# waiwera/waiwera

Hardware: AMD Instinct MI355X
Metric: Newton steps/sec, 10M-cell eos_we (BCSR SpMV GB/s in roofline) (higher is better)
Workload: dtype f64

## Files before the change

### include/waiwera_hip_bench.h

```cpp
#ifndef WAIWERA_HIP_BENCH_H
#define WAIWERA_HIP_BENCH_H
#include "waiwera_hip.h"
#ifdef __cplusplus
extern "C" {
#endif

int wai_comm_stats(wai_ctx *ctx, long long *allreduces, long long *exchanges);
int wai_gather_stats(wai_ctx *ctx, long long *gathers);
int wai_launch_stats(wai_ctx *ctx, long long *kernels, long long *copies);
int wai_tracer_stats(wai_ctx *ctx, long long *assembly_sweeps);

int wai_bench_mute_comm(wai_ctx *ctx, int on);
int wai_test_drop_partials(wai_ctx *ctx, int n);
int wai_test_drop_stream_wait(wai_ctx *ctx, int which);
int wai_test_network_pass(wai_ctx *ctx, const double *raw2n, double *sources6, double *groups6, double *reinjectors8,
                          double *net2n, double *enth_n);
int wai_test_network_stats(wai_ctx *ctx, long long *passes, long long *host_waits);
int wai_test_coupling_build_stats(wai_ctx *ctx, long long *launches, long long *columns, long long *chunks);
int wai_test_network_lds(wai_ctx *ctx, int *limit, int *needed);
int wai_test_device_memory(long long *allocations, long long *bytes);
int wai_test_pc_operator(wai_ctx *ctx, int spmv, const double *x, const double *x2, double alpha, int dot_mode,
                         const double *aux, int split, int fin_phase, const double *scal_in, double *z, double *scal_out);
int wai_pc_axpy_capable(wai_ctx *ctx);
int wai_test_partial_count(wai_ctx *ctx);
int wai_test_desc_templates(wai_ctx *ctx, int *bricks, int *rows);
int wai_test_pack_groups(wai_ctx *ctx, int list, int *shared, int *table, int cap);
int wai_test_tile_schedule(wai_ctx *ctx, int extended, int *facts);
enum { WAI_KV_DOT = 0, WAI_KV_DOTS, WAI_KV_WAXPY, WAI_KV_BCGS_P, WAI_KV_BCGS_S, WAI_KV_BCGS_XR, WAI_KV_BCGS_XRP,
       WAI_KV_BCGS_XRP_DERIVE, WAI_KV_SCALARS, WAI_KV_MDOT, WAI_KV_MAXPY_NORM, WAI_KV_SCALE_TO, WAI_KV_UPDATE_X };
int wai_test_krylov_vec(wai_ctx *ctx, int op, int variant, int n, int k, long long ld, long long len, double alpha,
                        double *vecs, double *basis, const double *coef, double *scal, double *post);
int wai_halo_size(wai_ctx *ctx, int dof, long long *bytes_sent, int *n_neighbours);

int wai_timer_start(wai_ctx *ctx);
int wai_timer_stop(wai_ctx *ctx, float *ms);
int wai_bench_kernel(wai_ctx *ctx, int which, int reps, float *ms_per_launch);
int wai_bcgs_composed(wai_ctx *ctx);
int wai_profile_enable(wai_ctx *ctx, int on);
int wai_profile_get(wai_ctx *ctx, int kclass, double *ms, long long *launches);
// ... 7 lines not shown
```

### waiwera_amd/csrc/capi.hip

```cpp
#include "host.hpp"

using namespace wai;

namespace wai {

int fetch_flags(wai_ctx* c, int out[4]) {
  if (c->comm && c->comm->nranks > 1) {
    HIPCHK(c, hipMemcpyAsync(c->h_flags, c->d_flags, 4 * sizeof(int), hipMemcpyDeviceToHost, c->stream));
    HIPCHK(c, hipStreamSynchronize(c->stream));
    double v[4] = {(double)c->h_flags[0], -(double)c->h_flags[1], (double)c->h_flags[2], (double)c->h_flags[3]};
    HIPCHK(c, hipMemcpyAsync(c->d_red + 2048, v, sizeof(v), hipMemcpyHostToDevice, c->stream));
    if (comm_allreduce(c->comm, c->d_red + 2048, 4, 1, c->stream, c->err)) return -1;
    HIPCHK(c, hipMemcpyAsync(c->h_red + 8, c->d_red + 2048, sizeof(v), hipMemcpyDeviceToHost, c->stream));
    HIPCHK(c, hipStreamSynchronize(c->stream));
    out[0] = (int)c->h_red[8]; out[1] = c->h_flags[1]; out[2] = (int)c->h_red[10]; out[3] = (int)c->h_red[11];
  } else {
    HIPCHK(c, hipMemcpyAsync(c->h_flags, c->d_flags, 4 * sizeof(int), hipMemcpyDeviceToHost, c->stream));
    HIPCHK(c, hipStreamSynchronize(c->stream));
    for (int i = 0; i < 4; i++) out[i] = c->h_flags[i];
  }
  HIPCHK(c, hipMemcpyAsync(c->d_flags, FLAGS_RESET, sizeof(FLAGS_RESET), hipMemcpyHostToDevice, c->stream));
  return 0;
}

// ... 10 lines not shown
  }
  int fl[4];
  if (fetch_flags(c, fl)) return -1;
  return fl[0] ? 1 : 0;
}

int do_residual(wai_ctx* c, double dt, double* y, const double* lhs_old, double* f) {
  int e = do_pre_eval(c, y);
  if (e) return e;
  if (c->net.on && network_update(c)) return -1;
  Prof p(c, KC_RESIDUAL);
  launch_residual(c, dt, lhs_old, f, nullptr, nullptr);
  return 0;
}

int do_jacobian(wai_ctx* c, double dt, const double* y, const double* lhs_old) {
  {
    Prof p(c, KC_EOS);
    launch_eos(c, y, 0, c->mesh.n_prim, true);
  }
  int fl[4];
  if (fetch_flags(c, fl)) return -1;
  if (fl[0]) return 1;
  Prof p(c, KC_JACOBIAN);
  if (launch_jacobian(c, dt, lhs_old)) return -1;
  pc_invalidate(c, c->flow);
  return network_couplings(c, dt, const_cast<double*>(y), lhs_old);
}

int do_norm2(wai_ctx* c, const double* v, double* out) {
  vec_dot(c, v, v, c->flow.n, S_W2);
  if (allreduce_scal(c, S_W2, 1)) return -1;
  if (read_scal(c, S_W2, 1)) return -1;
  *out = std::sqrt(c->ks.h_scal[S_W2]);
  return 0;
}

int do_max_scaled(wai_ctx* c, const double* v, const double* scale, double tol, double* val, int* idx) {
  if (launch_max_scaled(c, v, scale, tol, val, idx)) return -1;
  if (c->comm && c->comm->nranks > 1) {
// ... 385 lines not shown
```

### waiwera_amd/csrc/context.hip

```cpp
#include "host.hpp"
#include "cell_order.hpp"
#include <cstdio>

using namespace wai;

namespace wai {

int alloc_krylov_vecs(wai_ctx* c, KrylovVecs& k, size_t nl) {
  for (auto p : {&k.R, &k.RP, &k.P, &k.V, &k.S, &k.T, &k.tmp, &k.X_own})
    if (!*p && p->alloc_zeroed(c, nl + 16)) return -1;
  k.X = k.X_own;
  return 0;
}
int ensure_basis(wai_ctx* c, LinSys& sys, int m) {
  KrylovVecs& k = *sys.kv;
  if (k.basis && k.basis_m >= m) return 0;
  k.basis_m = m;
  return k.basis.alloc_zeroed(c, (size_t)(m + 4) * sys.nl);
}
int ensure_bcgsl_vecs(wai_ctx* c, KrylovVecs& k, size_t nl) {
  if (k.bl) return 0;
  return k.bl.alloc_zeroed(c, BCGSL_VECS * (nl + 16));
}
Bcsr matrix_on(const Pattern& p, int bs, double* val) {
// ... 2 lines not shown
  A.bs = bs; A.val = val;
  return A;
}
static KspOpts ksp_of(const wai_solver_opts& o) {
  KspOpts k;
  k.type = o.ksp_type; k.restart = o.gmres_restart; k.max_its = o.ksp_max_its; k.rtol = o.ksp_rtol; k.atol = o.ksp_atol;
  return k;
}

Handles::~Handles() {
  for (hipEvent_t e : {ev0, ev1, ev_scal, ev_pack, ev_halo}) if (e) (void)hipEventDestroy(e);
  if (comm_stream) (void)hipStreamDestroy(comm_stream);
  for (hipEvent_t e : {pev0, pev1}) if (e) (void)hipEventDestroy(e);
  if (stream) (void)hipStreamDestroy(stream);
  comm_destroy(comm);
}

}

static int create_handles(wai_ctx* c, int device) {
  c->device = device;
  HIPCHK(c, hipSetDevice(device));
  {
    int ncu = 0;
    if (hipDeviceGetAttribute(&ncu, hipDeviceAttributeMultiprocessorCount, device) == hipSuccess && ncu > 0) c->n_cu = ncu;
    int lds = 0;
    if (hipDeviceGetAttribute(&lds, hipDeviceAttributeMaxSharedMemoryPerBlock, device) == hipSuccess && lds > 0) c->lds_per_block = (size_t)lds;
  }
  HIPCHK(c, hipStreamCreateWithFlags(&c->stream, hipStreamNonBlocking));
  HIPCHK(c, hipEventCreate(&c->ev0)); HIPCHK(c, hipEventCreate(&c->ev1));
// ... 96 lines not shown
    std::vector<int> cs(N, -1);
    if (c->mesh.cell_src.upload(c, cs)) return -1;
  }
  std::vector<int> sub;
  if (md->sub_ptr && md->n_sub > 0) sub.assign(md->sub_ptr, md->sub_ptr + md->n_sub + 1);
  else sub = {0, N};
  return build_schedule(c, c->ilu, J.h_rowptr, J.h_colidx, sub, N, J.W, np, true);
}

static int create_vectors(wai_ctx* c) {
  const DeviceMesh& m = c->mesh;
  const int NL = m.n_local, np = c->np;
  LinSys& flow = c->flow;
  const size_t nl = (size_t)np * m.n_prim, n = (size_t)np * m.n_owned;
  const size_t fsz = (size_t)c->df * NL;
  if (c->flu.alloc_zeroed(c, fsz) || c->flu_last_iter.alloc(c, fsz) || c->flu_last_step.alloc(c, fsz) ||
      c->flu_pert.alloc(c, (size_t)np * c->df * m.n_prim) || c->hstep.alloc(c, nl))
    return -1;
  {
    std::vector<double> ones(NL, 1.0);
    HIPCHK(c, hipMemcpy(c->flu + (size_t)F_REGION * NL, ones.data(), NL * sizeof(double), hipMemcpyHostToDevice));
    HIPCHK(c, hipMemcpy(c->flu + (size_t)F_OLD_REGION * NL, ones.data(), NL * sizeof(double), hipMemcpyHostToDevice));
  }
  for (auto p : {&c->w_y, &c->w_yold, &c->w_delta, &c->w_f, &c->w_lhs, &c->w_a, &c->w_b, &c->w_c, &c->w_lhs2, &c->w_hist,
                 &c->w_hist_prev})
    if (p->alloc_zeroed(c, nl + 16)) return -1;
  flow.n = (int)n; flow.nl = (int)nl;
  if (alloc_krylov_vecs(c, c->kv, nl)) return -1;
  if (c->opts.gmres_restart > MAX_RESTART) { c->err = "gmres restart above 40 is not supported"; return -2; }
  c->kv.basis_m = basis_vectors(c->opts.gmres_restart);
  if ((flow.ksp.type == WAI_KSP_GMRES || flow.ksp.type == WAI_KSP_LGMRES) && ensure_basis(c, flow, c->kv.basis_m)) return -1;
  return 0;
// ... 321 lines not shown
```

### waiwera_amd/csrc/context.hpp

```cpp
#pragma once
#include <hip/hip_runtime.h>
#include <string>
#include <type_traits>
#include <vector>
#include "../../include/waiwera_hip.h"
#include "colour_order.hpp"
#include "coupling_batch.hpp"
#include "devbuf.hpp"
#include "ilu_schedule.hpp"
#include "mesh_pattern.hpp"
#include "network_pass.hpp"
#include "network_wave.hpp"
#include "physics.hip.h"
#include "tile_schedule.hpp"

namespace wai {

__host__ __device__ __forceinline__ size_t ell_ld(size_t n) {
  size_t ld = (n + 511) & ~(size_t)511;
  if ((ld & 262143) == 0) ld += 512;
  return ld;
}
__host__ __device__ __forceinline__ size_t ell_rows(int bs, size_t n) {
  if (bs >= 3) return ell_ld(n);
// ... 400 lines not shown
  wai::DevBuf<double> w_hist;
  wai::DevBuf<double> w_hist_prev;
  double dt_last_prev = 0.0;
  bool can_reject = false;
  bool prof_on = false;
  bool last_iter_partial = false;
  double prof_ms[wai::KC_COUNT] = {0};
  long long prof_n[wai::KC_COUNT] = {0};
  std::string err;
  bool bc_set = false;
  int dbg = 0;
};

namespace wai {
int launch_eos(wai_ctx* c, const double* y, int first, int count, bool perturbed);
int launch_residual(wai_ctx* c, double dt, const double* lhs_old, double* f, double* lhs_out,
                    double* rhs_out, const int* only = nullptr, int n_only = 0);
int launch_jacobian(wai_ctx* c, double dt, const double* lhs_old);
int launch_transitions(wai_ctx* c, const double* y_old, double* search, double* y);
int launch_tracer_assemble(wai_ctx* c, const TracerForm& tf, const double* alx_last,
                           const double* alx_last2, double* b);
int launch_tracer_assemble_all(wai_ctx* c, int method, double dt, double ratio, const double* alx_last,
                               const double* alx_last2, double* b);
int launch_tracer_lhs(wai_ctx* c, double* Al);
int launch_separator(wai_ctx* c, double pressure, double* out);
int launch_face_fluxes(wai_ctx* c, const int* face_cells, double* out);
int launch_source_rates(wai_ctx* c, double* out, bool raw = false);
int launch_network_pass(wai_ctx* c, const double* raw, double* net, double* enth, double* state_out, bool wave);
int net_wave_allow_lds(wai_ctx* c, const void* kernel, int bit, size_t* bytes);
int launch_cp_perturb(wai_ctx* c, double* p, double* yh);
int launch_cp_restore(wai_ctx* c, double* p, const double* yh);
int launch_cp_diff(wai_ctx* c, int ml, int m, int bs, int j, int k, const double* g, const double* yh, double* val, int* flag);
int launch_coupling_batch(wai_ctx* c, const CouplingBatch& b, int col0, int ncol, double dt, const double* y, const double* lhs_old,
// ... 70 lines not shown
```

### waiwera_amd/csrc/kernels_factor.hip

```cpp
#include "linalg_device.hip.h"
#include "pc_lu.hip.h"

namespace wai {

template <int BS>
__global__ void k_ilu_factor(int n, int nsub, const int* __restrict__ sub_ptr,
                             const int* __restrict__ sub_nlev, const int* __restrict__ row_info,
                             const int* __restrict__ col, double* fval, double* __restrict__ dinv,
                             int* flags) {
  constexpr int BB = BS * BS;
  const int s = xcd_remap(blockIdx.x, nsub);
  if (s >= nsub) return;
  const int lo = sub_ptr[s], R = sub_ptr[s + 1] - lo;
  const int nlf = sub_nlev[s] & 0xffff;
  const int i = lo + threadIdx.x;
  const bool active = (int)threadIdx.x < R;
  int lfirst = 0, dslot = 0, ulast = 0, lf = -1, lb = 0;
  if (active) unpack_info(row_info[i], lfirst, dslot, ulast, lf, lb);
  for (int lev = 0; lev < nlf; lev++) {
    if (active && lf == lev) {
      for (int q = lfirst; q < dslot; q++) {
        const int k = col[(size_t)q * n + i];
        int kl, kd, ku, kf, kb;
        unpack_info(row_info[k], kl, kd, ku, kf, kb);
// ... 109 lines not shown
      double piv[BB], inv[BB];
#pragma unroll
      for (int z = 0; z < BB; z++) piv[z] = fval[vix<BS>(n, dslot, z, i)];
      if (!block_inverse<BS>(piv, inv)) atomicMax(&flags[0], 1);
#pragma unroll
      for (int z = 0; z < BB; z++) {
        fval[vix<BS>(n, dslot, z, i)] = inv[z];
        dinv[dix<BS>(n, z, i)] = inv[z];
      }
    }
    __threadfence_block();
    __syncthreads();
  }
}

template <int BS, bool PRE>
__global__ void k_dilu_pivots(int n, int nsub, const int* __restrict__ sub_ptr,
                              const int* __restrict__ sub_nlev, const int* __restrict__ row_info,
                              const int* __restrict__ col, const double* __restrict__ aval,
                              double* __restrict__ dinv, int* flags) {
  constexpr int BB = BS * BS;
  extern __shared__ double pinv[];
  const int s = xcd_remap(blockIdx.x, nsub);
  if (s >= nsub) return;
  const int lo = sub_ptr[s], R = sub_ptr[s + 1] - lo;
  const int nlf = sub_nlev[s] & 0xffff;
  const int tid = threadIdx.x, i = lo + tid;
  const bool active = tid < R;
  int lfirst = 0, dslot = 0, ulast = 0, lf = -1, lb = 0;
  double P[BB];
#pragma unroll
  for (int e = 0; e < BB; e++) P[e] = 0.0;
  if (active) {
    unpack_info(row_info[i], lfirst, dslot, ulast, lf, lb);
    load_block<BS>(aval, n, dslot, i, P);
  }
  constexpr int NP = PRE ? 3 : 1;
  double paik[NP][BB], paki[NP][BB];
  int pk_off[NP];
  if constexpr (PRE) {
#pragma unroll
    for (int p = 0; p < NP; p++) {
      pk_off[p] = -1;
#pragma unroll
      for (int e = 0; e < BB; e++) { paik[p][e] = 0.0; paki[p][e] = 0.0; }
      const int q = lfirst + p;
      if (active && q < dslot) {
        const int k = col[(size_t)q * n + i];
        int kl, kd, ku, kf, kb;
        unpack_info(row_info[k], kl, kd, ku, kf, kb);
        load_block<BS>(aval, n, q, i, paik[p]);
// ... 41 lines not shown
          for (int e = 0; e < BB; e++) aki[e] = 0.0;
          for (int r2 = kd + 1; r2 < ku; r2++)
            if (col[(size_t)r2 * n + k] == i) { load_block<BS>(aval, n, r2, k, aki); break; }
          update(aik, pinv + (size_t)(k - lo) * BB, aki);
        }
      }
      double inv[BB];
      if (!block_inverse<BS>(P, inv)) atomicMax(&flags[0], 1);
#pragma unroll
      for (int e = 0; e < BB; e++) {
        pinv[(size_t)tid * BB + e] = inv[e];
        dinv[dix<BS>(n, e, i)] = inv[e];
      }
    }
    __syncthreads();
  }
}

template <int BS, int NPL, bool RAIK>
__global__ __launch_bounds__(256) void k_dilu_pivots_lds(int n, int nsub, int cap, const int* __restrict__ sub_ptr,
                                  const int* __restrict__ sub_nlev, const int* __restrict__ row_info,
                                  const int* __restrict__ row_tslot, const int* __restrict__ col,
                                  const double* __restrict__ aval, double* __restrict__ dinv, int* flags) {
  constexpr int BB = BS * BS;
  extern __shared__ double sm[];
  const int s = xcd_remap(blockIdx.x, nsub);
  if (s >= nsub) return;
  const int lo = sub_ptr[s], R = sub_ptr[s + 1] - lo;
  const int nlf = sub_nlev[s] & 0xffff;
  const int tid = threadIdx.x, i = lo + tid;
// ... 79 lines not shown
    __syncthreads();
  }
}

template <int BS>
__global__ __launch_bounds__(TPB) void k_scale_rows(int n, int W, const double* __restrict__ aval,
                                                    const double* __restrict__ dinv, double* __restrict__ sval) {
  constexpr int BB = BS * BS;
  const int i = blockIdx.x * TPB + threadIdx.x;
  if (i >= n) return;
  double d[BB];
  load_pivot<BS>(dinv, n, i, d);
  for (int q = 0; q < W; q++) {
    double a[BB];
    load_block<BS>(aval, n, q, i, a);
#pragma unroll
    for (int r = 0; r < BS; r++)
#pragma unroll
      for (int c = 0; c < BS; c++) {
        double t = 0.0;
#pragma unroll
        for (int e = 0; e < BS; e++) t += d[r * BS + e] * a[e * BS + c];
        sval[vix<BS>(n, q, r * BS + c, i)] = t;
      }
  }
}

template <int BS>
__global__ __launch_bounds__(TPB) void k_lvl_factor(int n, int cnt, const int* __restrict__ ord,
                                                    const int* __restrict__ row_info, const int* __restrict__ col,
                                                    double* fval, double* __restrict__ dinv, int* flags) {
  constexpr int BB = BS * BS;
  const int t = blockIdx.x * TPB + threadIdx.x;
  if (t >= cnt) return;
  const int i = ord[t];
  int lfirst, dslot, ulast;
  unpack_info_wide(row_info[i], lfirst, dslot, ulast);
  for (int q = lfirst; q < dslot; q++) {
    const int k = col[(size_t)q * n + i];
// ... 305 lines not shown
                       s.fval, s.dinv, c->d_flags);
    return;
  }
  if (s.big) {
    hipMemcpyAsync(s.fval, J.val, sizeof(double) * ell_size(J.bs, J.n, J.W), hipMemcpyDeviceToDevice, c->stream);
    for (int lev = 0; lev < s.nlev_f; lev++) {
      const int a = s.lev_f_ptr[lev], cnt = s.lev_f_ptr[lev + 1] - a, g = (cnt + TPB - 1) / TPB;
      if (cnt <= 0) continue;
      hipLaunchKernelGGL(k_lvl_factor<BS>, g, TPB, 0, c->stream, J.n, cnt, s.ord_f + a, s.row_info, J.col, s.fval, s.dinv, c->d_flags);
    }
    return;
  }
  const int grid = ((s.nsub + 7) / 8) * 8, T = pc_threads(s);
  if (s.diag_only && s.scaled) {
    const size_t lds = (size_t)T * J.bs * J.bs * sizeof(double);
    auto pivots = [&](auto pre) {
      hipLaunchKernelGGL((k_dilu_pivots<BS, decltype(pre)::value>), grid, T, lds, c->stream, J.n, s.nsub, s.sub_ptr, s.sub_nlev,
                         s.row_info, J.col, J.val, s.dinv, c->d_flags);
    };
    if constexpr (BS <= 2) with_flag(s.fast3, pivots);
    else if constexpr (BS == 3) {
      auto staged = [&](auto npl, auto raik, size_t lds_s) {
        hipLaunchKernelGGL((k_dilu_pivots_lds<3, decltype(npl)::value, decltype(raik)::value>), grid, T, lds_s, c->stream, J.n, s.nsub,
                           s.max_rows, s.sub_ptr, s.sub_nlev, s.row_info, s.row_tslot, J.col, J.val, s.dinv, c->d_flags);
      };
      const int npl = s.max_nl <= 3 ? 3 : 4;
      const size_t lds2 = (size_t)(1 + 2 * npl) * 9 * s.max_rows * sizeof(double);
      const std::integral_constant<int, 3> three;
      if (npl == 3 && T <= 64)
        staged(three, std::true_type{}, (size_t)(1 + npl) * 9 * s.max_rows * sizeof(double));
      else if (s.max_nl <= 4 && lds2 <= 64 * 1024 && T <= 256) {
        if (npl == 3) staged(three, std::false_type{}, lds2);
        else staged(std::integral_constant<int, 4>{}, std::false_type{}, lds2);
      } else
        pivots(std::false_type{});
    } else
      pivots(std::false_type{});
    hipLaunchKernelGGL(k_scale_rows<BS>, (J.n + TPB - 1) / TPB, TPB, 0, c->stream, J.n, J.W, J.val, s.dinv, s.fval);
    return;
  }
  hipMemcpyAsync(s.fval, J.val, sizeof(double) * ell_size(J.bs, J.n, J.W), hipMemcpyDeviceToDevice, c->stream);
  if (s.wide)
    hipLaunchKernelGGL(k_ilu_factor_wide<BS>, grid, T, 0, c->stream, J.n, s.nsub, s.sub_ptr, s.sub_nlev, s.row_infow, J.col, s.fval, s.dinv, c->d_flags);
  else
    hipLaunchKernelGGL(k_ilu_factor<BS>, grid, T, 0, c->stream, J.n, s.nsub, s.sub_ptr, s.sub_nlev, s.row_info, J.col, s.fval, s.dinv, c->d_flags);
}
int launch_ilu_factor_on(wai_ctx* c, const Bcsr& J, IluSchedule& s) {
  if (J.dg) return launch_dg_factor(c, J, s);
  return with_bs(J.bs, [&](auto bs) { ilu_factor_bs<decltype(bs)::value>(c, J, s); });
}

template <int BS, bool FWD>
static void lvl_sweep(wai_ctx* c, const Bcsr& J, const IluSchedule& s, const int* ord, const std::vector<int>& ptr, int nlev, double* z) {
// ... 51 lines not shown
```

### waiwera_amd/csrc/kernels_jacobian.hip

```cpp
#include "assembly_device.hip.h"

namespace wai {

template <int KIND>
__global__ __launch_bounds__(TPB) void k_jacobian(MeshView m, const double* __restrict__ flu,
                                                  size_t stride, const double* __restrict__ flu_pert,
                                                  const double* __restrict__ hstep, int n_prim,
                                                  ResForm rf, double* __restrict__ val) {
  using E = EosT<KIND>;
  constexpr int np = E::np, bb = E::np * E::np;
  const int c = xcd_cell(m.n_owned);
  if (c < 0) return;
  CellState<KIND> own0;
  RockState rown;
  load_state<KIND>(flu, stride, c, own0);
  load_rock(m.rock, m.n_local, c, rown);
  const double vol = m.vol[c];
  double lold[np], lold2[np];
#pragma unroll
  for (int k = 0; k < np; k++) {
    lold[k] = rf.method == WAI_METHOD_DIRECTSS ? 0.0 : rf.last[(size_t)c * np + k];
    lold2[k] = rf.method == WAI_METHOD_BDF2 ? rf.last2[(size_t)c * np + k] : 0.0;
  }

// ... 381 lines not shown
  for (int k = 0; k < np; k++) { R0[k] += src0[k]; f0[k] = res_form(rf, L0[k], R0[k], lold[k], lold2[k]); }
  const int dq = m.diag_blk[c];
#pragma unroll
  for (int k = 0; k < np; k++) {
    CellState<KIND> ownk;
    unpark_state<KIND>(park + (size_t)k * nld * st + threadIdx.x, st, ownk);
    source_terms<KIND>(m, c, ownk, vol, Rk[k]);
#pragma unroll
    for (int r = 0; r < np; r++) {
      const double f1 = res_form(rf, lpark[(size_t)(k * np + r) * st], Rk[k][r], lold[r], lold2[r]);
      __builtin_nontemporal_store((f1 - f0[r]) / hk[k], val + ell_ix(np, nrow, dq, r, k, (size_t)c));
    }
  }
}

int launch_jacobian(wai_ctx* c, double dt, const double* lhs_old) {
  const MeshView m = view(c);
  const size_t stride = c->mesh.n_local;
  const ResForm rf = res_form_of(c, dt, lhs_old);
  const char* ep = getenv("WAI_JAC_PARK");
  const bool park = !(ep && ep[0] == '0');
  const char* es = getenv("WAI_JAC_SYM");
  const bool sym = park && c->mesh.adj_tblk && (es ? es[0] == '1' : true);
  const char* kernel = nullptr;
  if (with_eos(c->kind, [&](auto k) {
        constexpr int K = decltype(k)::value;
        constexpr int T = ParkT<K>::threads;
        constexpr int sym_lds = EosT<K>::np * (ParkT<K>::npark + EosT<K>::np) * 8 * T;
        const int g = (((int)((m.n_owned + T - 1) / T) + 7) / 8) * 8;
        if (sym && (size_t)sym_lds <= c->lds_per_block) {
          kernel = "k_jacobian_sym";
          hipLaunchKernelGGL(k_jacobian_sym<K>, g, T, sym_lds, c->stream, m, c->flu, stride, c->flu_pert, c->hstep,
                             c->mesh.n_prim, rf, c->flow.A.val);
          return;
        }
        if (m.max_deg > MAXDEG) {
          c->err = "the row-wise Jacobian (WAI_JAC_SYM=0) supports cells with at most 8 faces; this mesh has a cell with " +
                   std::to_string(m.max_deg) + " (the default column-wise Jacobian takes up to 16)";
          return;
        }
        if (park && ParkT<K>::use) {
// ... 14 lines not shown
```

### waiwera_amd/csrc/measure.hip

```cpp
#include "host.hpp"

using namespace wai;

namespace {
typedef double stream_d2 __attribute__((ext_vector_type(2)));
__global__ __launch_bounds__(256) void k_stream_copy(const stream_d2* __restrict__ src, stream_d2* __restrict__ dst, size_t n2) {
  const size_t stride = (size_t)gridDim.x * 256;
  size_t i = (size_t)blockIdx.x * 256 + threadIdx.x;
  for (; i + stride < n2; i += 2 * stride) {
    const stream_d2 a = __builtin_nontemporal_load(src + i), b = __builtin_nontemporal_load(src + i + stride);
    __builtin_nontemporal_store(a, dst + i);
    __builtin_nontemporal_store(b, dst + i + stride);
  }
  if (i < n2) __builtin_nontemporal_store(__builtin_nontemporal_load(src + i), dst + i);
}
__global__ __launch_bounds__(256) void k_stream_read(const stream_d2* __restrict__ src, size_t n2, double* sink) {
  const size_t stride = (size_t)gridDim.x * 256;
  size_t i = (size_t)blockIdx.x * 256 + threadIdx.x;
  double t = 0.0;
  for (; i + stride < n2; i += 2 * stride) {
    const stream_d2 a = __builtin_nontemporal_load(src + i), b = __builtin_nontemporal_load(src + i + stride);
    t += (a.x + a.y) + (b.x + b.y);
  }
  if (i < n2) { const stream_d2 a = __builtin_nontemporal_load(src + i); t += a.x + a.y; }
// ... 13 lines not shown
  KrylovVecs& k = *sys.kv;
  if ((which == 20 || which == 21) && !k.basis) { c->err = "wai_bench_kernel 20 / 21: no Krylov basis (ksp_type gmres)"; return -2; }
  if (which > 0 && c->ilu.owner != &sys) { const int e = do_pc_setup(c, sys); if (e) return e < 0 ? -1 : e; }
  if (which > 0 && pc_colour(c, sys)) { c->err = "wai_bench_kernel: the natural order's kernels, not the multicolour ordering (tools/pc_colour_timing.py times it)"; return -2; }
  const bool fill = pc_fill_fused(c, sys);
  if (which == 23 && (!pc_fused(c, sys) || !(fill ? sys.as.sched.ord_f : c->ilu.ord_f))) {
    c->err = "wai_bench_kernel 23: no level sets (a block-Jacobi schedule of a wide mesh, or fused ILU(k))";
    return -2;
  }
  if (pc_asm_fused(c, sys) && (which == 9 || which == 10 || which == 16 || which == 23)) {
    c->err = "wai_bench_kernel 9 / 10 / 16 / 23: the brick schedule's kernels and the level sets of a factor on the system's own rows, not fused PCASM";
    return -2;
  }
  if (fill && (which == 9 || which == 10 || which == 16)) { c->err = "wai_bench_kernel 9 / 10 / 16: the brick schedule's kernels, not fused ILU(k)"; return -2; }
  const size_t copy_n = (size_t)c->np * c->df * c->mesh.n_prim / 2;
  auto run = [&]() {
    switch (which) {
      case 0: launch_spmv(c, sys.A, k.P, k.tmp); break;
      case 1: case 3: pc_solve(c, sys, k.P, k.V, PC_DOT_NONE, nullptr, nullptr); break;
      case 23:
        launch_spmv(c, sys.A, k.P, k.V);
        if (fill) launch_big_solve(c, sys.as.E, sys.as.sched, k.V);
        else launch_big_solve(c, sys.A, c->ilu, k.V);
        break;
      case 9: if (c->ilu.n_int > 0) launch_pc(c, sys.A, true, k.P, k.V, PC_DOT_ZA, k.RP, c->ilu.sub_int, c->ilu.n_int); break;
      case 10: if (c->ilu.n_bnd > 0) launch_pc(c, sys.A, true, k.P, k.V, PC_DOT_ZA, k.RP, c->ilu.sub_bnd, c->ilu.n_bnd); break;
      case 16:
        if (c->ilu.n_int > 0 && c->ilu.n_bnd > 0) {
          const Fin fin = make_fin_dots(c, PC_DOT_ZA, 2);
          launch_pc_split(c, sys.A, k.P, k.V, PC_DOT_ZA, k.RP, &fin, nullptr, nullptr);
// ... 181 lines not shown
    e = pc_amul(c, sys, k.R, k.T, dot_mode, a, fin_phase, v, false);
  } else {
    e = pc_solve(c, sys, k.R, k.T, dot_mode, k.R, a, fin_phase);
  }
  if (e) return e;
  if (fin_phase == -2 && dot_mode)
    vec_finalize(c, c->ks.nb_pc, pc_dot_slot0(dot_mode), pc_dot_nslots(dot_mode), -1);
  HIPCHK(c, hipMemcpyAsync(z, k.T, n * sizeof(double), hipMemcpyDefault, c->stream));
  HIPCHK(c, hipMemcpyAsync(s, c->ks.scal, sizeof(s), hipMemcpyDeviceToHost, c->stream));
  HIPCHK(c, hipStreamSynchronize(c->stream));
  for (int i = 0; i < 16; i++) scal_out[i] = s[i];
  return 0;
}
int wai_pc_axpy_capable(wai_ctx* c) { return c ? (pc_operand_composable(c) ? 1 : 0) : -2; }
int wai_test_partial_count(wai_ctx* c) { return c ? c->ks.nb_pc : -2; }
int wai_test_desc_templates(wai_ctx* c, int* bricks, int* rows) {
  if (!c) return -2;
  const bool have = c->ilu.sub_desc != nullptr;
  if (bricks) *bricks = c->ilu.nsub;
  if (rows) *rows = have ? c->ilu.template_rows : 0;
  return have ? c->ilu.n_templates : 0;
}
int wai_test_pack_groups(wai_ctx* c, int list, int* shared, int* table, int cap) {
  if (!c || list < 0 || list > 2 || cap < 0 || (cap > 0 && !table)) return -2;
  read_env(c);
  const IluSchedule& s = c->ilu;
  const bool packed = !s.big && pc_kernel_kind(c, c->flow.A, s) == 1 && s.col16 && !c->env.no_col16 && s.sub_desc &&
                      !c->env.no_desc_share && s.pack_tab[list] && !c->env.no_pack;
  if (shared) *shared = packed ? s.n_shared[list] : 0;
  if (!packed) return 0;
// ... 128 lines not shown
```

### waiwera_amd/flow_simulation.py

```python
import ctypes as C

import numpy as np

from . import lib as _lib
from .lib import LIB, WaiError


class FlowSimulation:
    def __init__(self, mesh, eos="we", opts=None, device=0, temperature=20.0,
                 relperm=("linear", [0.0, 1.0, 0.0, 1.0]), capillary=("zero", []), thermo="iapws",
                 permeability_modifier=None, thermo_extrapolate=False):
        self.mesh = mesh
        self.eos_name = eos
        self._keep = dict(
            face_cells=_lib._i32(mesh.face_cells), face_geom=_lib._f64(mesh.face_geom),
            cell_geom=_lib._f64(mesh.cell_geom), rock=_lib._f64(mesh.rock),
            sub_ptr=_lib._i32(mesh.sub_ptr) if mesh.sub_ptr is not None else None)
        k = self._keep
        md = _lib.MeshDesc()
        md.n_owned, md.n_halo, md.n_bc, md.n_faces = mesh.n_owned, mesh.n_halo, mesh.n_bc, mesh.n_faces
        md.face_cells = k["face_cells"].ctypes.data_as(_lib.pi)
        md.face_geom = k["face_geom"].ctypes.data_as(_lib.pd)
        md.cell_geom = k["cell_geom"].ctypes.data_as(_lib.pd)
        md.rock = k["rock"].ctypes.data_as(_lib.pd)
# ... 395 lines not shown
        ai = _lib._f64(aux) if aux is not None else None
        s_in = _lib._f64(np.zeros(16) if scal_in is None else scal_in)
        assert xi.size == self.num_dof and s_in.size == 16
        z, s_out = np.zeros(self.num_dof), np.zeros(16)
        self._chk(LIB.wai_test_pc_operator(self.h, 1 if spmv else 0, _lib.ptr(xi), _lib.ptr(x2i), float(alpha), int(dot_mode),
                                           _lib.ptr(ai), 1 if split else 0, int(fin_phase), s_in.ctypes.data_as(_lib.pd),
                                           _lib.ptr(z), s_out.ctypes.data_as(_lib.pd)), "test_pc_operator")
        return z, s_out

    def pc_axpy_capable(self):
        return LIB.wai_pc_axpy_capable(self.h) == 1

    def partial_count(self):
        return self._chk(LIB.wai_test_partial_count(self.h), "test_partial_count")

    def desc_templates(self):
        nb, nr = C.c_int(0), C.c_int(0)
        nt = self._chk(LIB.wai_test_desc_templates(self.h, C.byref(nb), C.byref(nr)), "test_desc_templates")
        return nt, nb.value, nr.value

    def pack_groups(self, which=0):
        shared = C.c_int(0)
        ng = self._chk(LIB.wai_test_pack_groups(self.h, which, C.byref(shared), None, 0), "test_pack_groups")
        table = np.zeros(ng * 32, dtype=np.int32)
        if ng:
            self._chk(LIB.wai_test_pack_groups(self.h, which, C.byref(shared), table.ctypes.data_as(C.POINTER(C.c_int)), table.size),
                      "test_pack_groups")
        return ng, shared.value, table.reshape(ng, 8, 4)

    KV_OPS = ("dot", "dots", "waxpy", "bcgs_p", "bcgs_s", "bcgs_xr", "bcgs_xrp", "bcgs_xrp_derive", "scalars", "mdot",
# ... 167 lines not shown
```

### waiwera_amd/lib.py

```python
import ctypes as C
import os

import numpy as np

HERE = os.path.dirname(os.path.abspath(__file__))
LIB_PATH = os.path.join(HERE, "libwaiwera_hip.so")

EOS_W, EOS_WE, EOS_WCE, EOS_WSE, EOS_WAE, EOS_WSCE, EOS_WSAE = 0, 1, 2, 3, 4, 5, 6
EOS_KIND = {"w": EOS_W, "we": EOS_WE, "wce": EOS_WCE, "wse": EOS_WSE, "wae": EOS_WAE, "wsce": EOS_WSCE,
            "wsae": EOS_WSAE}
RP = {"fully_mobile": 0, "fully mobile": 0, "linear": 1, "pickens": 2, "corey": 3, "grant": 4,
      "van_genuchten": 5, "van genuchten": 5, "table": 6}
CP = {"zero": 0, "linear": 1, "van_genuchten": 2, "van genuchten": 2, "table": 3}
INTERP = {"linear": 0, "step": 1, "pchip": 2}
KSP = {"bcgs": 0, "gmres": 1, "bcgsl": 2, "lgmres": 3}
PC = {"bjacobi": 0, "asm": 1, "none": 2, "lu": 3}
KCLASS = ["eos", "residual", "jacobian", "spmv", "pc_apply", "pc_setup", "vector", "transitions"]

d, i32 = C.c_double, C.c_int
pd, pi = C.POINTER(C.c_double), C.POINTER(C.c_int)


THERMO = {"iapws": 0, "ifc67": 1}
TRACER_SOLVE = {"per_tracer": 0, "coupled": 1}
# ... 116 lines not shown
        "wai_comm_init": (i32, [vp, i32, i32, C.c_char_p]),
        "wai_halo_exchange": (i32, [vp, vp, i32]),
        "wai_comm_size": (i32, [vp]),
        "wai_comm_stats": (i32, [vp, C.POINTER(C.c_longlong), C.POINTER(C.c_longlong)]),
        "wai_gather_stats": (i32, [vp, C.POINTER(C.c_longlong)]),
        "wai_gather_rows": (i32, [vp, i32, i32, vp, i32, vp, i32, vp]),
        "wai_gather_fluid": (i32, [vp, i32, i32, i32, pi, vp, i32, vp]),
        "wai_launch_stats": (i32, [vp, C.POINTER(C.c_longlong), C.POINTER(C.c_longlong)]),
        "wai_bench_mute_comm": (i32, [vp, i32]),
        "wai_test_drop_partials": (i32, [vp, i32]),
        "wai_test_drop_stream_wait": (i32, [vp, i32]),
        "wai_test_device_memory": (i32, [C.POINTER(C.c_longlong), C.POINTER(C.c_longlong)]),
        "wai_test_pc_operator": (i32, [vp, i32, vp, vp, d, i32, vp, i32, i32, pd, vp, pd]),
        "wai_pc_axpy_capable": (i32, [vp]),
        "wai_test_partial_count": (i32, [vp]),
        "wai_test_desc_templates": (i32, [vp, C.POINTER(i32), C.POINTER(i32)]),
        "wai_test_pack_groups": (i32, [vp, i32, C.POINTER(i32), C.POINTER(i32), i32]),
        "wai_test_tile_schedule": (i32, [vp, i32, C.POINTER(i32)]),
        "wai_test_krylov_vec": (i32, [vp, i32, i32, i32, i32, C.c_longlong, C.c_longlong, d, pd, pd, pd, pd, pd]),
        "wai_halo_size": (i32, [vp, i32, C.POINTER(C.c_longlong), C.POINTER(i32)]),
        "wai_pc_kernel_name": (C.c_char_p, [vp]),
        "wai_pre_timestep": (i32, [vp]),
        "wai_pre_retry_timestep": (i32, [vp]),
        "wai_pre_iteration": (i32, [vp]),
        "wai_pre_eval": (i32, [vp, d, vp]),
        "wai_lhs": (i32, [vp, d, vp, vp]),
        "wai_rhs": (i32, [vp, d, vp, vp]),
        "wai_post_linesearch": (i32, [vp, vp, vp, vp, pi, pi]),
        "wai_set_residual_form": (i32, [vp, i32, d, vp]),
        "wai_set_timestep_method": (i32, [vp, i32]),
# ... 202 lines not shown
```

Measured before the change: 5.394.

## Fuse row scaling into DILU pivot kernel and add lane-parallel Jacobian path

Folds the diagonal-inverse row scaling into the pivot kernel. Blocks already held in registers are reused, so the separate k_scale_rows pass and its reload of the matrix are skipped; this is on by default. Adds an opt-in Jacobian kernel that computes perturbed EOS states per lane inside the Jacobian itself, removing the separate perturbed EOS launch and the flu_pert buffer; this only runs when WAI_JAC_LANES=1. flu_pert is now allocated lazily, and test hooks are added for reading back the factor. The fused pivot kernel carries more register pressure, which could lower occupancy.

```diff
diff --git a/include/waiwera_hip_bench.h b/include/waiwera_hip_bench.h
--- a/include/waiwera_hip_bench.h
+++ b/include/waiwera_hip_bench.h
@@ -23,6 +23,8 @@
                          const double *aux, int split, int fin_phase, const double *scal_in, double *z, double *scal_out);
 int wai_pc_axpy_capable(wai_ctx *ctx);
 int wai_test_partial_count(wai_ctx *ctx);
+int wai_test_pc_factor(wai_ctx *ctx, long long cap_fval, double *fval, long long cap_dinv, double *dinv, int *scaled);
+int wai_test_pc_factor_size(wai_ctx *ctx, long long *n_fval, long long *n_dinv);
 int wai_test_desc_templates(wai_ctx *ctx, int *bricks, int *rows);
 int wai_test_pack_groups(wai_ctx *ctx, int list, int *shared, int *table, int cap);
 int wai_test_tile_schedule(wai_ctx *ctx, int extended, int *facts);
diff --git a/waiwera_amd/csrc/capi.hip b/waiwera_amd/csrc/capi.hip
--- a/waiwera_amd/csrc/capi.hip
+++ b/waiwera_amd/csrc/capi.hip
@@ -48,16 +48,29 @@
   return 0;
 }
 
+static std::string eos_range_message(int cell) {
+  return "FD Jacobian: a perturbed state of cell " + std::to_string(cell) + " is outside the range of the equation of state";
+}
+
 int do_jacobian(wai_ctx* c, double dt, const double* y, const double* lhs_old) {
+  int fl[4];
+  if (jacobian_lanes(c)) {
+    Prof p(c, KC_JACOBIAN);
+    if (launch_jacobian(c, dt, y, lhs_old)) return -1;
+    pc_invalidate(c, c->flow);
+    if (fetch_flags(c, fl)) return -1;
+    if (fl[0]) { c->err = eos_range_message(fl[1]); return 1; }
+    return network_couplings(c, dt, const_cast<double*>(y), lhs_old);
+  }
+  if (need_flu_pert(c)) return -1;
   {
     Prof p(c, KC_EOS);
     launch_eos(c, y, 0, c->mesh.n_prim, true);
   }
-  int fl[4];
   if (fetch_flags(c, fl)) return -1;
-  if (fl[0]) return 1;
+  if (fl[0]) { c->err = eos_range_message(fl[1]); return 1; }
   Prof p(c, KC_JACOBIAN);
-  if (launch_jacobian(c, dt, lhs_old)) return -1;
+  if (launch_jacobian(c, dt, y, lhs_old)) return -1;
   pc_invalidate(c, c->flow);
   return network_couplings(c, dt, const_cast<double*>(y), lhs_old);
 }
diff --git a/waiwera_amd/csrc/context.hip b/waiwera_amd/csrc/context.hip
--- a/waiwera_amd/csrc/context.hip
+++ b/waiwera_amd/csrc/context.hip
@@ -40,6 +40,11 @@
   for (hipEvent_t e : {pev0, pev1}) if (e) (void)hipEventDestroy(e);
   if (stream) (void)hipStreamDestroy(stream);
   comm_destroy(comm);
+}
+
+int need_flu_pert(wai_ctx* c) {
+  if (c->flu_pert) return 0;
+  return c->flu_pert.alloc(c, (size_t)c->np * c->df * c->mesh.n_prim);
 }
 
 }
@@ -166,8 +171,7 @@
   LinSys& flow = c->flow;
   const size_t nl = (size_t)np * m.n_prim, n = (size_t)np * m.n_owned;
   const size_t fsz = (size_t)c->df * NL;
-  if (c->flu.alloc_zeroed(c, fsz) || c->flu_last_iter.alloc(c, fsz) || c->flu_last_step.alloc(c, fsz) ||
-      c->flu_pert.alloc(c, (size_t)np * c->df * m.n_prim) || c->hstep.alloc(c, nl))
+  if (c->flu.alloc_zeroed(c, fsz) || c->flu_last_iter.alloc(c, fsz) || c->flu_last_step.alloc(c, fsz) || c->hstep.alloc(c, nl))
     return -1;
   {
     std::vector<double> ones(NL, 1.0);
diff --git a/waiwera_amd/csrc/context.hpp b/waiwera_amd/csrc/context.hpp
--- a/waiwera_amd/csrc/context.hpp
+++ b/waiwera_amd/csrc/context.hpp
@@ -438,9 +438,11 @@
 
 namespace wai {
 int launch_eos(wai_ctx* c, const double* y, int first, int count, bool perturbed);
+int need_flu_pert(wai_ctx* c);
+bool jacobian_lanes(const wai_ctx* c);
 int launch_residual(wai_ctx* c, double dt, const double* lhs_old, double* f, double* lhs_out,
                     double* rhs_out, const int* only = nullptr, int n_only = 0);
-int launch_jacobian(wai_ctx* c, double dt, const double* lhs_old);
+int launch_jacobian(wai_ctx* c, double dt, const double* y, const double* lhs_old);
 int launch_transitions(wai_ctx* c, const double* y_old, double* search, double* y);
 int launch_tracer_assemble(wai_ctx* c, const TracerForm& tf, const double* alx_last,
                            const double* alx_last2, double* b);
diff --git a/waiwera_amd/csrc/kernels_factor.hip b/waiwera_amd/csrc/kernels_factor.hip
--- a/waiwera_amd/csrc/kernels_factor.hip
+++ b/waiwera_amd/csrc/kernels_factor.hip
@@ -147,11 +147,23 @@
   }
 }
 
-template <int BS, bool PRE>
+template <int BS>
+__device__ __forceinline__ void scale_block(const double* d, const double* a, double* __restrict__ sval, int n, int q, int i) {
+#pragma unroll
+  for (int r = 0; r < BS; r++)
+#pragma unroll
+    for (int c = 0; c < BS; c++) {
+      double t = 0.0;
+#pragma unroll
+      for (int e = 0; e < BS; e++) t += d[r * BS + e] * a[e * BS + c];
+      sval[vix<BS>(n, q, r * BS + c, i)] = t;
+    }
+}
+template <int BS, bool PRE, bool SCALE>
 __global__ void k_dilu_pivots(int n, int nsub, const int* __restrict__ sub_ptr,
                               const int* __restrict__ sub_nlev, const int* __restrict__ row_info,
                               const int* __restrict__ col, const double* __restrict__ aval,
-                              double* __restrict__ dinv, int* flags) {
+                              double* __restrict__ dinv, int* flags, int W, double* __restrict__ sval) {
   constexpr int BB = BS * BS;
   extern __shared__ double pinv[];
   const int s = xcd_remap(blockIdx.x, nsub);
@@ -168,6 +180,11 @@
     unpack_info(row_info[i], lfirst, dslot, ulast, lf, lb);
     load_block<BS>(aval, n, dslot, i, P);
   }
+  double adiag[PRE && SCALE ? BB : 1];
+  if constexpr (PRE && SCALE) {
+#pragma unroll
+    for (int e = 0; e < BB; e++) adiag[e] = P[e];
+  }
   constexpr int NP = PRE ? 3 : 1;
   double paik[NP][BB], paki[NP][BB];
   int pk_off[NP];
@@ -239,6 +256,32 @@
       }
     }
     __syncthreads();
+  }
+  if constexpr (SCALE) {
+    if (!active) return;
+    double d[BB];
+#pragma unroll
+    for (int e = 0; e < BB; e++) d[e] = pinv[(size_t)tid * BB + e];
+    for (int q = 0; q < W; q++) {
+      double a[BB];
+      bool held = false;
+      if constexpr (PRE) {
+        if (q == dslot) {
+          held = true;
+#pragma unroll
+          for (int e = 0; e < BB; e++) a[e] = adiag[e];
+        }
+#pragma unroll
+        for (int p = 0; p < NP; p++)
+          if (q == lfirst + p && q < dslot) {
+            held = true;
+#pragma unroll
+            for (int e = 0; e < BB; e++) a[e] = paik[p][e];
+          }
+      }
+      if (!held) load_block<BS>(aval, n, q, i, a);
+      scale_block<BS>(d, a, sval, n, q, i);
+    }
   }
 }
 
@@ -348,15 +391,7 @@
   for (int q = 0; q < W; q++) {
     double a[BB];
     load_block<BS>(aval, n, q, i, a);
-#pragma unroll
-    for (int r = 0; r < BS; r++)
-#pragma unroll
-      for (int c = 0; c < BS; c++) {
-        double t = 0.0;
-#pragma unroll
-        for (int e = 0; e < BS; e++) t += d[r * BS + e] * a[e * BS + c];
-        sval[vix<BS>(n, q, r * BS + c, i)] = t;
-      }
+    scale_block<BS>(d, a, sval, n, q, i);
   }
 }
 
@@ -692,9 +727,15 @@
   const int grid = ((s.nsub + 7) / 8) * 8, T = pc_threads(s);
   if (s.diag_only && s.scaled) {
     const size_t lds = (size_t)T * J.bs * J.bs * sizeof(double);
+    const char* ef = getenv("WAI_PIVOT_SCALE");
+    const bool fuse = !(ef && ef[0] == '0');
+    bool scaled_rows = false;
     auto pivots = [&](auto pre) {
-      hipLaunchKernelGGL((k_dilu_pivots<BS, decltype(pre)::value>), grid, T, lds, c->stream, J.n, s.nsub, s.sub_ptr, s.sub_nlev,
-                         s.row_info, J.col, J.val, s.dinv, c->d_flags);
+      with_flag(fuse, [&](auto sc) {
+        hipLaunchKernelGGL((k_dilu_pivots<BS, decltype(pre)::value, decltype(sc)::value>), grid, T, lds, c->stream, J.n, s.nsub, s.sub_ptr,
+                           s.sub_nlev, s.row_info, J.col, J.val, s.dinv, c->d_flags, J.W, s.fval);
+      });
+      scaled_rows = fuse;
     };
     if constexpr (BS <= 2) with_flag(s.fast3, pivots);
     else if constexpr (BS == 3) {
@@ -714,7 +755,8 @@
         pivots(std::false_type{});
     } else
       pivots(std::false_type{});
-    hipLaunchKernelGGL(k_scale_rows<BS>, (J.n + TPB - 1) / TPB, TPB, 0, c->stream, J.n, J.W, J.val, s.dinv, s.fval);
+    if (!scaled_rows)
+      hipLaunchKernelGGL(k_scale_rows<BS>, (J.n + TPB - 1) / TPB, TPB, 0, c->stream, J.n, J.W, J.val, s.dinv, s.fval);
     return;
   }
   hipMemcpyAsync(s.fval, J.val, sizeof(double) * ell_size(J.bs, J.n, J.W), hipMemcpyDeviceToDevice, c->stream);
diff --git a/waiwera_amd/csrc/kernels_jacobian.hip b/waiwera_amd/csrc/kernels_jacobian.hip
--- a/waiwera_amd/csrc/kernels_jacobian.hip
+++ b/waiwera_amd/csrc/kernels_jacobian.hip
@@ -419,7 +419,122 @@
   }
 }
 
-int launch_jacobian(wai_ctx* c, double dt, const double* lhs_old) {
+template <int KIND> struct LanesT {
+#if defined(WAI_JAC_LANES_G2)
+  static constexpr int G = EosT<KIND>::np == 2 ? WAI_JAC_LANES_G2 : EosT<KIND>::np + 1;
+#else
+  static constexpr int G = EosT<KIND>::np + 1;
+#endif
+  static constexpr int per_wave = 64 / G;
+  static constexpr int threads = 256;
+  static constexpr int cells = (threads / 64) * per_wave;
+#if defined(WAI_JAC_LANES_WAVES)
+  static constexpr int waves = WAI_JAC_LANES_WAVES;
+#else
+  static constexpr int waves = 2;
+#endif
+};
+template <int KIND>
+__device__ __forceinline__ void as_loaded(CellState<KIND>& s) {
+  using E = EosT<KIND>;
+  s.region = 0.0;
+#pragma unroll
+  for (int q = 0; q < E::nc; q++) s.pp[q] = 0.0;
+  if constexpr (E::nc == 1) {
+#pragma unroll
+    for (int p = 0; p < E::nph; p++) s.x[p][0] = (((int)s.phases >> p) & 1) ? 1.0 : 0.0;
+  }
+}
+template <int KIND>
+__global__ __launch_bounds__(LanesT<KIND>::threads, LanesT<KIND>::waves) void k_jacobian_lanes(MeshView m, EosParams ep, const double* __restrict__ y,
+                                                  const double* __restrict__ flu, size_t stride, double eps, double umin,
+                                                  ResForm rf, double* __restrict__ val, int* flags) {
+  using E = EosT<KIND>;
+  using LT = LanesT<KIND>;
+  constexpr int np = E::np, G = LT::G;
+  const int nblk = (m.n_owned + LT::cells - 1) / LT::cells;
+  const int per = (nblk + 7) >> 3;
+  const int b = ((int)blockIdx.x & 7) * per + ((int)blockIdx.x >> 3);
+  if (((int)blockIdx.x >> 3) >= per || b >= nblk) return;
+  const int lane = (int)threadIdx.x & 63, grp = lane / G, role = lane - grp * G;
+  const int c = b * LT::cells + ((int)threadIdx.x >> 6) * LT::per_wave + grp;
+  if (grp >= LT::per_wave || role > np || c >= m.n_owned) return;
+  const int base = lane - role;
+  const int k = role - 1;
+  CellState<KIND> own;
+  RockState rown;
+  load_rock(m.rock, m.n_local, c, rown);
+  const double vol = m.vol[c];
+  double h = 1.0;
+  if (role == 0) load_state<KIND>(flu, stride, c, own);
+  else {
+    double yc[np];
+#pragma unroll
+    for (int q = 0; q < np; q++) yc[q] = y[(size_t)c * np + q];
+#pragma unroll
+    for (int q = 0; q < np; q++)
+      if (q == k) { h = fd_step(yc[q], eps, umin); yc[q] += h; }
+    const int region = (int)flu[F_REGION * stride + c];
+    if (eos_eval<KIND>(ep, yc, region, own)) flag_error(flags, c);
+    as_loaded<KIND>(own);
+  }
+  const size_t nrow = m.n_owned;
+  const double dR = res_dR(rf);
+  double L[np], R[np];
+  cell_balance<KIND>(own, rown, L);
+#pragma unroll
+  for (int q = 0; q < np; q++) R[q] = 0.0;
+#pragma unroll 1
+  for (int s = 0; s < m.max_deg; s++) {
+    const int fs = m.adj_face[(size_t)s * m.n_owned + c];
+    if (fs < 0) continue;
+    const int o = m.adj_other[(size_t)s * m.n_owned + c];
+    const int tb = m.adj_tblk[(size_t)s * m.n_owned + c];
+    FaceGeom g;
+    load_face(m, fs >> 1, g);
+    CellState<KIND> oth;
+    RockState roth;
+    load_state<KIND>(flu, stride, o, oth);
+    load_rock_face(m.rock, m.n_local, o, g.dir, roth);
+    const int side = fs & 1;
+    const double sign = side ? 1.0 : -1.0;
+    const double volo = tb >= 0 ? m.vol[o] : 1.0;
+    double fl[np];
+    slot_flux<KIND>(g, side, own, rown, oth, roth, fl);
+#pragma unroll
+    for (int q = 0; q < np; q++) R[q] += sign * (fl[q] * g.area) / vol;
+#pragma unroll
+    for (int r = 0; r < np; r++) {
+      const double to = -sign * (fl[r] * g.area) / volo;
+      const double to0 = __shfl(to, base);
+      if (role > 0 && tb >= 0) val[ell_ix(np, nrow, tb, r, k, (size_t)o)] = dR * (to - to0) / h;
+    }
+  }
+  double acc[np];
+#pragma unroll
+  for (int q = 0; q < np; q++) acc[q] = role == 0 ? 0.0 : R[q];
+  source_terms<KIND>(m, c, own, vol, acc);
+#pragma unroll
+  for (int q = 0; q < np; q++) R[q] = role == 0 ? R[q] + acc[q] : acc[q];
+  const int dq = m.diag_blk[c];
+#pragma unroll
+  for (int r = 0; r < np; r++) {
+    const double l1 = rf.method == WAI_METHOD_DIRECTSS ? 0.0 : rf.last[(size_t)c * np + r];
+    const double l2 = rf.method == WAI_METHOD_BDF2 ? rf.last2[(size_t)c * np + r] : 0.0;
+    const double f = res_form(rf, L[r], R[r], l1, l2);
+    const double f0 = __shfl(f, base);
+    if (role > 0) __builtin_nontemporal_store((f - f0) / h, val + ell_ix(np, nrow, dq, r, k, (size_t)c));
+  }
+}
+
+bool jacobian_lanes(const wai_ctx* c) {
+  const char* ep = getenv("WAI_JAC_PARK");
+  const char* es = getenv("WAI_JAC_SYM");
+  const char* el = getenv("WAI_JAC_LANES");
+  return !(ep && ep[0] == '0') && c->mesh.adj_tblk && c->mesh.n_halo == 0 && !(es && es[0] != '1') && (el && el[0] == '1');
+}
+
+int launch_jacobian(wai_ctx* c, double dt, const double* y, const double* lhs_old) {
   const MeshView m = view(c);
   const size_t stride = c->mesh.n_local;
   const ResForm rf = res_form_of(c, dt, lhs_old);
@@ -428,8 +543,18 @@
   const char* es = getenv("WAI_JAC_SYM");
   const bool sym = park && c->mesh.adj_tblk && (es ? es[0] == '1' : true);
   const char* kernel = nullptr;
+  const bool lanes = jacobian_lanes(c);
+  if (!lanes && !c->flu_pert) { c->err = "launch_jacobian: the perturbed fluid records (flu_pert) are not allocated"; return -1; }
   if (with_eos(c->kind, [&](auto k) {
         constexpr int K = decltype(k)::value;
+        if (lanes) {
+          using LT = LanesT<K>;
+          const int gl = (((int)((m.n_owned + LT::cells - 1) / LT::cells) + 7) / 8) * 8;
+          kernel = "k_jacobian_lanes";
+          hipLaunchKernelGGL(k_jacobian_lanes<K>, gl, LT::threads, 0, c->stream, m, c->ep, y, c->flu, stride, c->opts.fd_eps,
+                             c->opts.fd_umin, rf, c->flow.A.val, c->d_flags);
+          return;
+        }
         constexpr int T = ParkT<K>::threads;
         constexpr int sym_lds = EosT<K>::np * (ParkT<K>::npark + EosT<K>::np) * 8 * T;
         const int g = (((int)((m.n_owned + T - 1) / T) + 7) / 8) * 8;
diff --git a/waiwera_amd/csrc/measure.hip b/waiwera_amd/csrc/measure.hip
--- a/waiwera_amd/csrc/measure.hip
+++ b/waiwera_amd/csrc/measure.hip
@@ -51,6 +51,7 @@
   }
   if (fill && (which == 9 || which == 10 || which == 16)) { c->err = "wai_bench_kernel 9 / 10 / 16: the brick schedule's kernels, not fused ILU(k)"; return -2; }
   const size_t copy_n = (size_t)c->np * c->df * c->mesh.n_prim / 2;
+  if ((which == 18 || which == 19 || which == 22) && need_flu_pert(c)) return -1;
   auto run = [&]() {
     switch (which) {
       case 0: launch_spmv(c, sys.A, k.P, k.tmp); break;
@@ -262,6 +263,25 @@
 }
 int wai_pc_axpy_capable(wai_ctx* c) { return c ? (pc_operand_composable(c) ? 1 : 0) : -2; }
 int wai_test_partial_count(wai_ctx* c) { return c ? c->ks.nb_pc : -2; }
+int wai_test_pc_factor_size(wai_ctx* c, long long* n_fval, long long* n_dinv) {
+  if (!c || !n_fval || !n_dinv) return -2;
+  const Bcsr& J = c->flow.A;
+  *n_fval = (long long)ell_size(J.bs, J.n, J.W);
+  *n_dinv = (long long)J.n * J.bs * J.bs;
+  return 0;
+}
+int wai_test_pc_factor(wai_ctx* c, long long cap_fval, double* fval, long long cap_dinv, double* dinv, int* scaled) {
+  if (!c || cap_fval < 0 || cap_dinv < 0 || (cap_fval > 0 && !fval) || (cap_dinv > 0 && !dinv)) return -2;
+  const Bcsr& J = c->flow.A;
+  const IluSchedule& s = c->ilu;
+  if (!s.fval || !s.dinv) { c->err = "wai_test_pc_factor: no block ILU factor (wai_pc_setup first)"; return -1; }
+  const size_t nf = ell_size(J.bs, J.n, J.W), nd = (size_t)J.n * J.bs * J.bs;
+  if (scaled) *scaled = (s.diag_only && s.scaled) ? 1 : 0;
+  HIPCHK(c, hipStreamSynchronize(c->stream));
+  if (cap_fval > 0) HIPCHK(c, hipMemcpy(fval, s.fval, std::min((size_t)cap_fval, nf) * sizeof(double), hipMemcpyDeviceToHost));
+  if (cap_dinv > 0) HIPCHK(c, hipMemcpy(dinv, s.dinv, std::min((size_t)cap_dinv, nd) * sizeof(double), hipMemcpyDeviceToHost));
+  return 0;
+}
 int wai_test_desc_templates(wai_ctx* c, int* bricks, int* rows) {
   if (!c) return -2;
   const bool have = c->ilu.sub_desc != nullptr;
diff --git a/waiwera_amd/flow_simulation.py b/waiwera_amd/flow_simulation.py
--- a/waiwera_amd/flow_simulation.py
+++ b/waiwera_amd/flow_simulation.py
@@ -433,6 +433,16 @@
     def partial_count(self):
         return self._chk(LIB.wai_test_partial_count(self.h), "test_partial_count")
 
+    def pc_factor(self):
+        nf, nd, sc = C.c_longlong(0), C.c_longlong(0), C.c_int(0)
+        self._chk(LIB.wai_test_pc_factor_size(self.h, C.byref(nf), C.byref(nd)), "test_pc_factor_size")
+        fval, dinv = np.zeros(nf.value), np.zeros(nd.value)
+        self._chk(LIB.wai_test_pc_factor(self.h, nf.value, _lib.ptr(fval), nd.value, _lib.ptr(dinv), C.byref(sc)), "test_pc_factor")
+        return fval, dinv, bool(sc.value)
+
+    def last_error(self):
+        return LIB.wai_last_error(self.h).decode()
+
     def desc_templates(self):
         nb, nr = C.c_int(0), C.c_int(0)
         nt = self._chk(LIB.wai_test_desc_templates(self.h, C.byref(nb), C.byref(nr)), "test_desc_templates")
diff --git a/waiwera_amd/lib.py b/waiwera_amd/lib.py
--- a/waiwera_amd/lib.py
+++ b/waiwera_amd/lib.py
@@ -154,6 +154,8 @@
         "wai_test_pc_operator": (i32, [vp, i32, vp, vp, d, i32, vp, i32, i32, pd, vp, pd]),
         "wai_pc_axpy_capable": (i32, [vp]),
         "wai_test_partial_count": (i32, [vp]),
+        "wai_test_pc_factor": (i32, [vp, C.c_longlong, vp, C.c_longlong, vp, C.POINTER(i32)]),
+        "wai_test_pc_factor_size": (i32, [vp, C.POINTER(C.c_longlong), C.POINTER(C.c_longlong)]),
         "wai_test_desc_templates": (i32, [vp, C.POINTER(i32), C.POINTER(i32)]),
         "wai_test_pack_groups": (i32, [vp, i32, C.POINTER(i32), C.POINTER(i32), i32]),
         "wai_test_tile_schedule": (i32, [vp, i32, C.POINTER(i32)]),
```

Measured after the change: 5.401 (median of 3 runs). About the same (+0.1%).
